# advimman/lama

Hardware: NVIDIA H100
Metric: images/sec FFCResNetGenerator @512x512 bs32 (higher is better)
Workload: dtype bf16x3(f32 accumulate)

## Files before the change

lama_b200/csrc/fft_plane_cg.cu:

```cuda
#include <stdint.h>

#include "common.cuh"
#include "fft_plane_cg.cuh"

namespace ffcb {
namespace {

using namespace fftc;

struct CgArgs {
  const float* in;  long long in_sg, in_sb;  unsigned in_sy, in_sx;
  void* spec;       long long sp_sg, sp_sb;  unsigned sp_sy, sp_sx; long long sp_lo;
  void* out;        long long out_sg, out_sb; unsigned out_sy, out_sx; long long out_lo;
  float scale;
  int hints;
  int sp_tiled;
  int out_tiled;
};

__device__ __forceinline__ uint32_t smem_addr(const void* p) { return (uint32_t)__cvta_generic_to_shared(p); }

__device__ __forceinline__ void cp_async16(uint32_t dst, const void* src, uint64_t pol) {
  asm volatile("cp.async.cg.shared.global.L2::cache_hint [%0], [%1], 16, %2;" ::"r"(dst), "l"(src), "l"(pol) : "memory");
}
__device__ __forceinline__ void cp_async_wait_all() { asm volatile("cp.async.wait_all;" ::: "memory"); }

template <int N, bool DENSE>
__global__ void __launch_bounds__(kCgThreads, CgCfg<N>::ctas_per_sm) rfft2_plane_cg_kernel(CgArgs a) {
  using Cfg = CgCfg<N>;
  constexpr unsigned WF = N / 2 + 1;
  const unsigned in_sy = DENSE ? 4u * N : a.in_sy, in_sx = DENSE ? 4u : a.in_sx;
  const unsigned sp_sy = DENSE ? 8u * WF : a.sp_sy, sp_sx = DENSE ? 8u : a.sp_sx;
  extern __shared__ __align__(16) float smem_all[];
  const int set = threadIdx.x / Cfg::set_threads, tid = threadIdx.x % Cfg::set_threads;
  const int group = blockIdx.x * Cfg::sets + set;
  float* smem = smem_all + set * Cfg::set_floats;
  float2* S = reinterpret_cast<float2*>(smem);
  {
    const float* src = a.in + (long long)group * a.in_sg + (long long)blockIdx.y * a.in_sb;
    const uint32_t base = smem_addr(smem);
    const uint64_t pol_in = l2_policy(a.hints ? 1 : 0);
#pragma unroll 8
    for (int i = 0; i < Cfg::px_iters; ++i) {
      int y, x;
      cg_pixel_slot<N>(tid, i, y, x);
      cp_async16(base + 4u * (unsigned)cg_real_idx<N>(y, x, 0), src + ((unsigned)y * in_sy + (unsigned)x * in_sx),
                 pol_in);
    }
    cp_async_wait_all();
  }
  float2* NQ = reinterpret_cast<float2*>(smem_all + Cfg::sets * Cfg::set_floats) + set * (N * 4);
  float2 v[N];
#pragma unroll 1
  for (int pass = 0; pass < 2; ++pass) {
    __syncthreads();
    if (pass == 0) {
      cg_fwd_rows_load<N>(tid, v, [&](int i) { return *reinterpret_cast<const float2*>(smem + i); });
      __syncwarp();
    } else {
      cg_fwd_cols_load<N>(tid, v, [&](int i2) { return S[i2]; });
    }
    RegFft<N>::template run<false>(v);
    if (pass == 0) {
      cg_fwd_rows_post<N>(tid, v, [&](int i2, float4 q) { *reinterpret_cast<float4*>(S + i2) = q; });
    } else {
      auto put = [&](int ky, int kx, int c, float2 z) {
        if (kx == N / 2) NQ[ky * 4 + c] = z;
        else S[cg_cplx_idx<N>(ky, kx, c)] = z;
      };
      if (tid < 32) cg_fwd_cols_post<N, true>(tid, v, put);
      else cg_fwd_cols_post<N, false>(tid, v, put);
    }
  }
  __syncthreads();
  {
    unsigned short* hi = reinterpret_cast<unsigned short*>(a.spec) + (long long)group * a.sp_sg +
                         (long long)blockIdx.y * a.sp_sb;
    const float scale = a.scale;
    const uint64_t pol_sp = l2_policy(a.hints ? 2 : 0);
    int ky, kx;
    cg_spec_pos0<N>(tid, ky, kx);
    unsigned short* tbase = reinterpret_cast<unsigned short*>(a.spec) + (long long)group * 1024;
    long long m = (long long)blockIdx.y * Cfg::positions + tid;
#pragma unroll 1
    for (int i = 0; i < Cfg::pos_iters; ++i) {
      if (ky < N) {
        const float4* src = kx == N / 2 ? reinterpret_cast<const float4*>(NQ + ky * 4)
                                        : reinterpret_cast<const float4*>(S + cg_cplx_idx<N>(ky, kx, 0));
        const float4 q0 = src[0], q1 = src[1];
        uint4 h, l;
        const float2 z0 = cscale(make_float2(q0.x, q0.y), scale), z1 = cscale(make_float2(q0.z, q0.w), scale);
        const float2 z2 = cscale(make_float2(q1.x, q1.y), scale), z3 = cscale(make_float2(q1.z, q1.w), scale);
        split_pair(z0.x, z0.y, h.x, l.x);
        split_pair(z1.x, z1.y, h.y, l.y);
        split_pair(z2.x, z2.y, h.z, l.z);
        split_pair(z3.x, z3.y, h.w, l.w);
        unsigned short* dst = a.sp_tiled ? tbase + ((m >> 7) * a.sp_sg + (m & 127) * 8)
                                         : hi + ((unsigned)ky * sp_sy + (unsigned)kx * sp_sx);
        st_hint_u4(dst, h, pol_sp);
        st_hint_u4(dst + a.sp_lo, l, pol_sp);
      }
      cg_spec_pos_next<N>(ky, kx);
      m += Cfg::set_threads;
    }
  }
}

template <int N, bool HAS_RES, bool OUT_SPLIT, bool DENSE>
__global__ void __launch_bounds__(kCgThreads, CgCfg<N>::ctas_per_sm) irfft2_plane_cg_kernel(CgArgs a) {
  using Cfg = CgCfg<N>;
  constexpr unsigned WF = N / 2 + 1;
  const unsigned in_sy = DENSE ? 4u * N : a.in_sy, in_sx = DENSE ? 4u : a.in_sx;
  const unsigned sp_sy = DENSE ? 8u * WF : a.sp_sy, sp_sx = DENSE ? 8u : a.sp_sx;
  const unsigned out_sy = DENSE ? (OUT_SPLIT ? 8u : 4u) * N : a.out_sy, out_sx = DENSE ? (OUT_SPLIT ? 8u : 4u) : a.out_sx;
  extern __shared__ __align__(16) float smem_all[];
  const int set = threadIdx.x / Cfg::set_threads, tid = threadIdx.x % Cfg::set_threads;
  const int group = blockIdx.x * Cfg::sets + set;
  float* smem = smem_all + set * Cfg::set_floats;
  float2* S = reinterpret_cast<float2*>(smem);
  {
    const float* sp = reinterpret_cast<const float*>(a.spec) + (long long)group * a.sp_sg +
                      (long long)blockIdx.y * a.sp_sb + 2 * (tid & 3);
    const uint64_t pol_sp = l2_policy(a.hints ? 1 : 0);
    auto ldz = [&](int ky, int kx) { return ld_hint_f2(sp + ((unsigned)ky * sp_sy + (unsigned)kx * sp_sx), pol_sp); };
    float2 v[N];
#pragma unroll 1
    for (int pass = 0; pass < 2; ++pass) {
      if (pass == 0) {
        if (tid < 32) cg_inv_cols_load<N, true>(tid, v, ldz);
        else cg_inv_cols_load<N, false>(tid, v, ldz);
      } else {
        __syncthreads();
        cg_inv_rows_load<N>(tid, v, [&](int i2) { return *reinterpret_cast<const float4*>(S + i2); });
        __syncwarp();
      }
      RegFft<N>::template run<true>(v);
      if (pass == 0) cg_inv_cols_post<N>(tid, v, [&](int i2, float2 z) { S[i2] = z; });
      else cg_inv_rows_post<N>(tid, v, [&](int i, float2 z) { *reinterpret_cast<float2*>(smem + i) = z; });
    }
  }
  __syncthreads();
  {
    const float* res = HAS_RES ? a.in + (long long)group * a.in_sg + (long long)blockIdx.y * a.in_sb : nullptr;
    const float scale = a.scale;
    const uint64_t pol_res = l2_policy(a.hints ? 1 : 0), pol_out = l2_policy(a.hints ? 2 : 0);
#pragma unroll 1
    for (int i0 = 0; i0 < Cfg::px_iters; i0 += 8) {
      float4 q[8];
#pragma unroll
      for (int j = 0; j < 8; ++j) {
        int y, x;
        cg_pixel_slot<N>(tid, i0 + j, y, x);
        q[j] = HAS_RES ? ld_hint_f4(res + ((unsigned)y * in_sy + (unsigned)x * in_sx), pol_res)
                       : make_float4(0.f, 0.f, 0.f, 0.f);
      }
#pragma unroll
      for (int j = 0; j < 8; ++j) {
        int y, x;
        cg_pixel_slot<N>(tid, i0 + j, y, x);
        const float4 v = *reinterpret_cast<const float4*>(smem + cg_real_idx<N>(y, x, 0));
        const float r0 = fmaf(v.x, scale, q[j].x), r1 = fmaf(v.y, scale, q[j].y);
        const float r2 = fmaf(v.z, scale, q[j].z), r3 = fmaf(v.w, scale, q[j].w);
        if constexpr (OUT_SPLIT) {
          unsigned short* hi;
          if (a.out_tiled) {
            const long long m = ((long long)blockIdx.y * N + y) * N + x;
            hi = reinterpret_cast<unsigned short*>(a.out) + ((m >> 7) * a.out_sg + (long long)(group >> 1) * 1024 +
                                                               (m & 127) * 8 + 4 * (group & 1));
          } else {
            hi = reinterpret_cast<unsigned short*>(a.out) + (long long)(group >> 1) * a.out_sg +
                 (long long)blockIdx.y * a.out_sb + 4 * (group & 1) + ((unsigned)y * out_sy + (unsigned)x * out_sx);
          }
          unsigned h0, l0, h1, l1;
          split_pair(r0, r1, h0, l0);
          split_pair(r2, r3, h1, l1);
          st_hint_v2(hi, make_uint2(h0, h1), pol_out);
          st_hint_v2(hi + a.out_lo, make_uint2(l0, l1), pol_out);
        } else {
          float* op = reinterpret_cast<float*>(a.out) + (long long)group * a.out_sg +
                      (long long)blockIdx.y * a.out_sb + ((unsigned)y * out_sy + (unsigned)x * out_sx);
          st_hint_f4(op, make_float4(r0, r1, r2, r3), pol_out);
        }
      }
    }
  }
}

bool offsets_fit(const ffcb_tensor* t) { return t->sy > 0 && t->sx > 0 && 64 * t->sy + 64 * t->sx < (1LL << 31); }

bool plane_ok(int h, int w, int c) { return (h == 64 && w == 64) || (h == 32 && w == 32 && c % 8 == 0); }

bool real_cg4(const ffcb_tensor* t) {
  return t->cg == 4 && t->fmt == FFCB_F32 && plane_ok(t->H, t->W, t->C) && t->sx % 4 == 0 && t->sy % 4 == 0 &&
         t->sb % 4 == 0 && t->sg % 4 == 0 && ((uintptr_t)t->ptr % 16) == 0 && offsets_fit(t) && t->B <= 65535;
}

}

bool plane64_cg_fwd_eligible(const ffcb_tensor* in, const ffcb_tensor* spec) {
  if (!(real_cg4(in) && spec->cg == 8 && spec->fmt == FFCB_BF16X2 && spec->lo_off % 8 == 0 &&
        ((uintptr_t)spec->ptr % 16) == 0))
    return false;
  if (spec->tile) return spec->tile == 128 && spec->sg % 8 == 0;
  return spec->sx % 8 == 0 && spec->sy % 8 == 0 && spec->sb % 8 == 0 && spec->sg % 8 == 0 && offsets_fit(spec);
}

bool plane64_cg_inv_eligible(const ffcb_tensor* spec, const ffcb_tensor* residual, const ffcb_tensor* out) {
  if (!(spec->cg == 8 && spec->fmt == FFCB_F32 && spec->sx % 2 == 0 && spec->sy % 2 == 0 && spec->sb % 2 == 0 &&
        spec->sg % 2 == 0 && ((uintptr_t)spec->ptr % 8) == 0 && offsets_fit(spec) && plane_ok(out->H, out->W, out->C) &&
        out->B <= 65535))
    return false;
  if (residual && residual->ptr && !real_cg4(residual)) return false;
  if (out->fmt == FFCB_BF16X2) {
    if (!(out->cg == 8 && out->lo_off % 4 == 0 && ((uintptr_t)out->ptr % 8) == 0 && out->C % 8 == 0)) return false;
    if (out->tile) return out->tile == 128 && out->sg % 4 == 0;
    return out->sx % 4 == 0 && out->sy % 4 == 0 && out->sb % 4 == 0 && out->sg % 4 == 0 && offsets_fit(out);
  }
  return real_cg4(out);
}

template <int N, bool DENSE>
static int launch_fwd_cg(const CgArgs& a, int groups, int batch, cudaStream_t stream) {
  using Cfg = CgCfg<N>;
  FFCB_CUDA(cudaFuncSetAttribute(rfft2_plane_cg_kernel<N, DENSE>, cudaFuncAttributeMaxDynamicSharedMemorySize,
                                 Cfg::fwd_smem_bytes));
  dim3 grid(groups / Cfg::sets, batch);
  rfft2_plane_cg_kernel<N, DENSE><<<grid, kCgThreads, Cfg::fwd_smem_bytes, stream>>>(a);
  FFCB_LAUNCH_CHECK("rfft2_plane_cg_kernel");
  return FFCB_OK;
}

static bool dense_real(const ffcb_tensor* t, int cg) { return t->sx == cg && t->sy == (int64_t)t->W * cg; }

int rfft2_plane64_cg(const ffcb_tensor* in, const ffcb_tensor* spec, cudaStream_t stream) {
  CgArgs a{};
  a.in = reinterpret_cast<const float*>(in->ptr);
  a.in_sg = in->sg; a.in_sb = in->sb; a.in_sy = (unsigned)in->sy; a.in_sx = (unsigned)in->sx;
  a.spec = spec->ptr; a.sp_sg = spec->sg; a.sp_sb = spec->sb; a.sp_sy = (unsigned)spec->sy; a.sp_sx = (unsigned)spec->sx;
  a.sp_lo = spec->lo_off;
  a.sp_tiled = spec->tile != 0;
  a.scale = 1.0f / (float)in->H;
  a.hints = l2_hints_enabled() ? 1 : 0;
  const bool dense = dense_real(in, 4) && (spec->tile != 0 || dense_real(spec, 8));
  if (in->H == 64)
    return dense ? launch_fwd_cg<64, true>(a, in->C / 4, in->B, stream) : launch_fwd_cg<64, false>(a, in->C / 4, in->B, stream);
  return dense ? launch_fwd_cg<32, true>(a, in->C / 4, in->B, stream) : launch_fwd_cg<32, false>(a, in->C / 4, in->B, stream);
}

template <int N, bool HAS_RES, bool OUT_SPLIT, bool DENSE>
static int launch_inv_cg(const CgArgs& a, int groups, int batch, cudaStream_t stream) {
  using Cfg = CgCfg<N>;
  FFCB_CUDA(cudaFuncSetAttribute(irfft2_plane_cg_kernel<N, HAS_RES, OUT_SPLIT, DENSE>,
                                 cudaFuncAttributeMaxDynamicSharedMemorySize, Cfg::smem_bytes));
  dim3 grid(groups / Cfg::sets, batch);
  irfft2_plane_cg_kernel<N, HAS_RES, OUT_SPLIT, DENSE><<<grid, kCgThreads, Cfg::smem_bytes, stream>>>(a);
  FFCB_LAUNCH_CHECK("irfft2_plane_cg_kernel");
  return FFCB_OK;
}

template <int N, bool DENSE>
static int dispatch_inv_cg(const CgArgs& a, int groups, int batch, bool has_res, bool split, cudaStream_t stream) {
  if (has_res)
    return split ? launch_inv_cg<N, true, true, DENSE>(a, groups, batch, stream)
                 : launch_inv_cg<N, true, false, DENSE>(a, groups, batch, stream);
  return split ? launch_inv_cg<N, false, true, DENSE>(a, groups, batch, stream)
               : launch_inv_cg<N, false, false, DENSE>(a, groups, batch, stream);
}

int irfft2_plane64_cg(const ffcb_tensor* spec, const ffcb_tensor* residual, const ffcb_tensor* out,
                      cudaStream_t stream) {
  const bool has_res = residual && residual->ptr;
  CgArgs a{};
  if (has_res) {
    a.in = reinterpret_cast<const float*>(residual->ptr);
    a.in_sg = residual->sg; a.in_sb = residual->sb; a.in_sy = (unsigned)residual->sy; a.in_sx = (unsigned)residual->sx;
  }
  a.spec = spec->ptr; a.sp_sg = spec->sg; a.sp_sb = spec->sb; a.sp_sy = (unsigned)spec->sy; a.sp_sx = (unsigned)spec->sx;
  a.out = out->ptr; a.out_sg = out->sg; a.out_sb = out->sb; a.out_sy = (unsigned)out->sy; a.out_sx = (unsigned)out->sx;
  a.out_lo = out->lo_off;
  a.out_tiled = out->tile != 0;
  a.scale = 1.0f / (float)out->H;
  a.hints = l2_hints_enabled() ? 1 : 0;
  const bool split = out->fmt == FFCB_BF16X2;
  const bool dense = dense_real(spec, 8) && (out->tile != 0 || dense_real(out, split ? 8 : 4)) &&
                     (!has_res || dense_real(residual, 4));
  if (out->H == 64)
    return dense ? dispatch_inv_cg<64, true>(a, out->C / 4, out->B, has_res, split, stream)
                 : dispatch_inv_cg<64, false>(a, out->C / 4, out->B, has_res, split, stream);
  return dense ? dispatch_inv_cg<32, true>(a, out->C / 4, out->B, has_res, split, stream)
               : dispatch_inv_cg<32, false>(a, out->C / 4, out->B, has_res, split, stream);
}

}
```

lama_b200/csrc/fft_plane_cg.cuh:

```cuda
#pragma once
#include "fft_core.cuh"

namespace ffcb {
namespace fftc {

constexpr int kCgThreads = 128;
template <int N> struct CgCfg {
  static constexpr int set_threads = 2 * N;
  static constexpr int sets = kCgThreads / set_threads;
  static constexpr int set_floats = N * N * 4;
  static constexpr int smem_bytes = sets * set_floats * 4;
  static constexpr int px_iters = N * N / set_threads;
  static constexpr int positions = N * (N / 2 + 1);
  static constexpr int pos_iters = (positions + set_threads - 1) / set_threads;
  static constexpr int fwd_smem_bytes = smem_bytes + sets * N * 4 * 8;
  static constexpr int ctas_per_sm = N == 64 ? 3 : 4;
};
constexpr int kCgSmemBytes = CgCfg<64>::smem_bytes;

template <int N> FFCB_HD int cg_real_idx(int y, int x, int c) { return y * (4 * N) + ((x ^ (y & 7)) << 2) + c; }
template <int N> FFCB_HD int cg_cplx_idx(int y, int k, int c) { return y * (2 * N) + ((k ^ (y & 3)) << 2) + c; }


template <int N, class Load>
FFCB_HD void cg_fwd_rows_load(int tid, float2* v, Load&& ld2) {
  const int cp = tid & 1, y = tid >> 1;
#pragma unroll
  for (int x = 0; x < N; ++x) v[x] = ld2(cg_real_idx<N>(y, x, 2 * cp));
}

template <int N, class Store>
FFCB_HD void cg_fwd_rows_post(int tid, const float2* v, Store&& st4) {
  using F = RegFft<N>;
  const int cp = tid & 1, y = tid >> 1;
#pragma unroll
  for (int k = 0; k < N / 2; ++k) {
    const float2 zk = v[F::at(k)], zm = v[F::at((N - k) & (N - 1))];
    const float2 cm = make_float2(zm.x, -zm.y), df = csub(zk, cm);
    float2 a = cscale(cadd(zk, cm), 0.5f);
    float2 b = cscale(make_float2(df.y, -df.x), 0.5f);
    if (k == 0) {
      const float2 zn = v[F::at(N / 2)];
      a = make_float2(zk.x, zn.x);
      b = make_float2(zk.y, zn.y);
    }
    st4(cg_cplx_idx<N>(y, k, 2 * cp), make_float4(a.x, a.y, b.x, b.y));
  }
}

template <int N, class Load, class Sync, class Store>
FFCB_HD void cg_fwd_rows(int tid, Load&& ld2, Sync&& sync, Store&& st4) {
  float2 v[N];
  cg_fwd_rows_load<N>(tid, v, ld2);
  sync();
  RegFft<N>::template run<false>(v);
  cg_fwd_rows_post<N>(tid, v, st4);
}

template <int N, class Load>
FFCB_HD void cg_fwd_cols_load(int tid, float2* v, Load&& ld) {
  const int c = tid & 3, kx = tid >> 2;
#pragma unroll
  for (int y = 0; y < N; ++y) v[y] = ld(cg_cplx_idx<N>(y, kx, c));
}

template <int N, bool MAYBE_PACKED, class Emit>
FFCB_HD void cg_fwd_cols_post(int tid, const float2* v, Emit&& emit) {
  using F = RegFft<N>;
  const int c = tid & 3, kx = tid >> 2;
  const bool packed = MAYBE_PACKED && kx == 0;
#pragma unroll
  for (int k = 0; k < N; ++k) {
    const float2 wk = v[F::at(k)];
    if constexpr (MAYBE_PACKED) {
      const float2 wm = v[F::at((N - k) & (N - 1))];
      const float2 cm = make_float2(wm.x, -wm.y), df = csub(wk, cm);
      const float2 x0 = cscale(cadd(wk, cm), 0.5f);
      const float2 x32 = cscale(make_float2(df.y, -df.x), 0.5f);
      emit(k, kx, c, packed ? x0 : wk);
      if (packed) emit(k, N / 2, c, x32);
    } else {
      emit(k, kx, c, wk);
    }
  }
}

template <int N, bool MAYBE_PACKED, class Load, class Emit>
FFCB_HD void cg_fwd_cols(int tid, Load&& ld, Emit&& emit) {
  float2 v[N];
  cg_fwd_cols_load<N>(tid, v, ld);
  RegFft<N>::template run<false>(v);
  cg_fwd_cols_post<N, MAYBE_PACKED>(tid, v, emit);
}

template <int N, bool MAYBE_PACKED, class Load>
FFCB_HD void cg_inv_cols_load(int tid, float2* v, Load&& ld) {
  const int kx = tid >> 2;
  const bool packed = MAYBE_PACKED && kx == 0;
#pragma unroll
  for (int k = 0; k < N; ++k) v[k] = ld(k, kx);
  if constexpr (MAYBE_PACKED) {
#pragma unroll
    for (int k = 0; k <= N / 2; ++k) {
      const int m = (N - k) & (N - 1);
      const float2 a = v[k], b = v[m];
      float2 cc = make_float2(0.f, 0.f), d = make_float2(0.f, 0.f);
      if (packed) {
        cc = ld(k, N / 2);
        d = (m != k) ? ld(m, N / 2) : cc;
      }
      const float2 h0 = cscale(cadd(a, make_float2(b.x, -b.y)), 0.5f);
      const float2 h32 = cscale(cadd(cc, make_float2(d.x, -d.y)), 0.5f);
      const float2 ih = make_float2(-h32.y, h32.x);
      const float2 lo = cadd(h0, ih), hi = csub(h0, ih);
      v[k] = packed ? lo : a;
      if (m != k) v[m] = packed ? make_float2(hi.x, -hi.y) : b;
    }
  }
}

template <int N, class Store>
FFCB_HD void cg_inv_cols_post(int tid, const float2* v, Store&& st) {
  using F = RegFft<N>;
  const int c = tid & 3, kx = tid >> 2;
#pragma unroll
  for (int y = 0; y < N; ++y) st(cg_cplx_idx<N>(y, kx, c), v[F::at(y)]);
}

template <int N, bool MAYBE_PACKED, class Load, class Store>
FFCB_HD void cg_inv_cols(int tid, Load&& ld, Store&& st) {
  float2 v[N];
  cg_inv_cols_load<N, MAYBE_PACKED>(tid, v, ld);
  RegFft<N>::template run<true>(v);
  cg_inv_cols_post<N>(tid, v, st);
}

template <int N, class Load>
FFCB_HD void cg_inv_rows_load(int tid, float2* v, Load&& ld4) {
  const int cp = tid & 1, y = tid >> 1;
#pragma unroll
  for (int k = 0; k < N / 2; ++k) {
    const float4 q = ld4(cg_cplx_idx<N>(y, k, 2 * cp));
    if (k == 0) {
      v[0] = make_float2(q.x, q.z);
      v[N / 2] = make_float2(q.y, q.w);
    } else {
      const float2 x1 = make_float2(q.x, q.y), ix2 = make_float2(-q.w, q.z), dd = csub(x1, ix2);
      v[k] = cadd(x1, ix2);
      v[N - k] = make_float2(dd.x, -dd.y);
    }
  }
}

template <int N, class Store>
FFCB_HD void cg_inv_rows_post(int tid, const float2* v, Store&& st2) {
  using F = RegFft<N>;
  const int cp = tid & 1, y = tid >> 1;
#pragma unroll
  for (int x = 0; x < N; ++x) st2(cg_real_idx<N>(y, x, 2 * cp), v[F::at(x)]);
}

template <int N, class Load, class Sync, class Store>
FFCB_HD void cg_inv_rows(int tid, Load&& ld4, Sync&& sync, Store&& st2) {
  float2 v[N];
  cg_inv_rows_load<N>(tid, v, ld4);
  sync();
  RegFft<N>::template run<true>(v);
  cg_inv_rows_post<N>(tid, v, st2);
}

template <int N>
FFCB_HD void cg_spec_pos0(int tid, int& ky, int& kx) {
  ky = tid / (N / 2 + 1);
  kx = tid % (N / 2 + 1);
}
template <int N>
FFCB_HD void cg_spec_pos_next(int& ky, int& kx) {
  constexpr int WF = N / 2 + 1, T = 2 * N;
  kx += T % WF;
  ky += T / WF;
  if (kx >= WF) { kx -= WF; ++ky; }
}

template <int N>
FFCB_HD void cg_pixel_slot(int tid, int i, int& y, int& x) {
  const int p = i * CgCfg<N>::set_threads + tid;
  y = p / N;
  x = p % N;
}

}
}
```

Baseline: 329.5.

## Make inverse plane FFT kernel persistent with L2 bulk prefetch of next spectrum

Turns the inverse FFT plane kernel into a persistent grid-stride loop over (group-set, batch) units, capped at SMs × CTAs-per-SM. Each iteration issues cp.async.bulk L2 prefetches for the current residual and the next unit's spectrum, aiming to hide global-memory latency. An extra __syncthreads is added before the shared-memory column store so buffers can be reused across iterations. The trade-off is more barriers and a fixed grid that can load-balance poorly, and the prefetch adds memory traffic on a path that may already be bandwidth-bound.

```diff
diff --git a/lama_b200/csrc/fft_plane_cg.cu b/lama_b200/csrc/fft_plane_cg.cu
--- a/lama_b200/csrc/fft_plane_cg.cu
+++ b/lama_b200/csrc/fft_plane_cg.cu
@@ -16,6 +16,9 @@
   int hints;
   int sp_tiled;
   int out_tiled;
+  int pf_spec;
+  int gx_count;
+  int units;
 };
 
 __device__ __forceinline__ uint32_t smem_addr(const void* p) { return (uint32_t)__cvta_generic_to_shared(p); }
@@ -24,6 +27,9 @@
   asm volatile("cp.async.cg.shared.global.L2::cache_hint [%0], [%1], 16, %2;" ::"r"(dst), "l"(src), "l"(pol) : "memory");
 }
 __device__ __forceinline__ void cp_async_wait_all() { asm volatile("cp.async.wait_all;" ::: "memory"); }
+__device__ __forceinline__ void prefetch_l2(const void* p, int bytes) {
+  asm volatile("cp.async.bulk.prefetch.L2.global [%0], %1;" ::"l"(p), "r"(bytes) : "memory");
+}
 
 template <int N, bool DENSE>
 __global__ void __launch_bounds__(kCgThreads, CgCfg<N>::ctas_per_sm) rfft2_plane_cg_kernel(CgArgs a) {
@@ -115,71 +121,98 @@
   const unsigned out_sy = DENSE ? (OUT_SPLIT ? 8u : 4u) * N : a.out_sy, out_sx = DENSE ? (OUT_SPLIT ? 8u : 4u) : a.out_sx;
   extern __shared__ __align__(16) float smem_all[];
   const int set = threadIdx.x / Cfg::set_threads, tid = threadIdx.x % Cfg::set_threads;
-  const int group = blockIdx.x * Cfg::sets + set;
   float* smem = smem_all + set * Cfg::set_floats;
   float2* S = reinterpret_cast<float2*>(smem);
-  {
-    const float* sp = reinterpret_cast<const float*>(a.spec) + (long long)group * a.sp_sg +
-                      (long long)blockIdx.y * a.sp_sb + 2 * (tid & 3);
-    const uint64_t pol_sp = l2_policy(a.hints ? 1 : 0);
-    auto ldz = [&](int ky, int kx) { return ld_hint_f2(sp + ((unsigned)ky * sp_sy + (unsigned)kx * sp_sx), pol_sp); };
-    float2 v[N];
-#pragma unroll 1
-    for (int pass = 0; pass < 2; ++pass) {
-      if (pass == 0) {
-        if (tid < 32) cg_inv_cols_load<N, true>(tid, v, ldz);
-        else cg_inv_cols_load<N, false>(tid, v, ldz);
-      } else {
-        __syncthreads();
-        cg_inv_rows_load<N>(tid, v, [&](int i2) { return *reinterpret_cast<const float4*>(S + i2); });
-        __syncwarp();
-      }
-      RegFft<N>::template run<true>(v);
-      if (pass == 0) cg_inv_cols_post<N>(tid, v, [&](int i2, float2 z) { S[i2] = z; });
-      else cg_inv_rows_post<N>(tid, v, [&](int i, float2 z) { *reinterpret_cast<float2*>(smem + i) = z; });
-    }
-  }
-  __syncthreads();
-  {
-    const float* res = HAS_RES ? a.in + (long long)group * a.in_sg + (long long)blockIdx.y * a.in_sb : nullptr;
-    const float scale = a.scale;
-    const uint64_t pol_res = l2_policy(a.hints ? 1 : 0), pol_out = l2_policy(a.hints ? 2 : 0);
-#pragma unroll 1
-    for (int i0 = 0; i0 < Cfg::px_iters; i0 += 8) {
-      float4 q[8];
+  auto spec_of = [&](int u) {
+    int gx, b;
+    cg_unit(u, a.gx_count, gx, b);
+    return reinterpret_cast<const float*>(a.spec) + (long long)(gx * Cfg::sets + set) * a.sp_sg + (long long)b * a.sp_sb;
+  };
+#pragma unroll 1
+  for (int u = blockIdx.x; u < a.units; u += gridDim.x) {
+    const int next = u + gridDim.x;
+    int gx, b;
+    cg_unit(u, a.gx_count, gx, b);
+    const int group = gx * Cfg::sets + set;
+    const float* res = HAS_RES ? a.in + (long long)group * a.in_sg + (long long)b * a.in_sb : nullptr;
+    if (DENSE && tid < kCgPrefetchChunks) {
+      int off, bytes;
+      if (HAS_RES) {
+        cg_prefetch_chunk(tid, Cfg::real_set_bytes, off, bytes);
+        prefetch_l2(reinterpret_cast<const char*>(res) + off, bytes);
+      }
+      if (a.pf_spec && next < a.units) {
+        cg_prefetch_chunk(tid, Cfg::spec_set_bytes, off, bytes);
+        prefetch_l2(reinterpret_cast<const char*>(spec_of(next)) + off, bytes);
+      }
+    }
+    {
+      const float* sp0 = spec_of(u) + 2 * (tid & 3);
+      const uint64_t pol_sp = l2_policy(a.hints ? 1 : 0);
+      float2 v[N];
+#pragma unroll 1
+      for (int pass = 0; pass < 2; ++pass) {
+        if (pass == 0) {
+          const float* sp = sp0;
+          asm volatile("" : "+l"(sp));
+          auto ldz = [&](int ky, int kx) { return ld_hint_f2(sp + ((unsigned)ky * sp_sy + (unsigned)kx * sp_sx), pol_sp); };
+          if (tid < 32) cg_inv_cols_load<N, true>(tid, v, ldz);
+          else cg_inv_cols_load<N, false>(tid, v, ldz);
+        } else {
+          __syncthreads();
+          cg_inv_rows_load<N>(tid, v, [&](int i2) { return *reinterpret_cast<const float4*>(S + i2); });
+          __syncwarp();
+        }
+        RegFft<N>::template run<true>(v);
+        if (pass == 0) {
+          __syncthreads();
+          cg_inv_cols_post<N>(tid, v, [&](int i2, float2 z) { S[i2] = z; });
+        } else {
+          cg_inv_rows_post<N>(tid, v, [&](int i, float2 z) { *reinterpret_cast<float2*>(smem + i) = z; });
+        }
+      }
+    }
+    __syncthreads();
+    {
+      const float scale = a.scale;
+      const uint64_t pol_res = l2_policy(a.hints ? 1 : 0), pol_out = l2_policy(a.hints ? 2 : 0);
+#pragma unroll 1
+      for (int i0 = 0; i0 < Cfg::px_iters; i0 += 8) {
+        float4 q[8];
 #pragma unroll
-      for (int j = 0; j < 8; ++j) {
-        int y, x;
-        cg_pixel_slot<N>(tid, i0 + j, y, x);
-        q[j] = HAS_RES ? ld_hint_f4(res + ((unsigned)y * in_sy + (unsigned)x * in_sx), pol_res)
-                       : make_float4(0.f, 0.f, 0.f, 0.f);
-      }
+        for (int j = 0; j < 8; ++j) {
+          int y, x;
+          cg_pixel_slot<N>(tid, i0 + j, y, x);
+          q[j] = HAS_RES ? ld_hint_f4(res + ((unsigned)y * in_sy + (unsigned)x * in_sx), pol_res)
+                         : make_float4(0.f, 0.f, 0.f, 0.f);
+        }
 #pragma unroll
-      for (int j = 0; j < 8; ++j) {
-        int y, x;
-        cg_pixel_slot<N>(tid, i0 + j, y, x);
-        const float4 v = *reinterpret_cast<const float4*>(smem + cg_real_idx<N>(y, x, 0));
-        const float r0 = fmaf(v.x, scale, q[j].x), r1 = fmaf(v.y, scale, q[j].y);
-        const float r2 = fmaf(v.z, scale, q[j].z), r3 = fmaf(v.w, scale, q[j].w);
-        if constexpr (OUT_SPLIT) {
-          unsigned short* hi;
-          if (a.out_tiled) {
-            const long long m = ((long long)blockIdx.y * N + y) * N + x;
-            hi = reinterpret_cast<unsigned short*>(a.out) + ((m >> 7) * a.out_sg + (long long)(group >> 1) * 1024 +
-                                                               (m & 127) * 8 + 4 * (group & 1));
+        for (int j = 0; j < 8; ++j) {
+          int y, x;
+          cg_pixel_slot<N>(tid, i0 + j, y, x);
+          const float4 v = *reinterpret_cast<const float4*>(smem + cg_real_idx<N>(y, x, 0));
+          const float r0 = fmaf(v.x, scale, q[j].x), r1 = fmaf(v.y, scale, q[j].y);
+          const float r2 = fmaf(v.z, scale, q[j].z), r3 = fmaf(v.w, scale, q[j].w);
+          if constexpr (OUT_SPLIT) {
+            unsigned short* hi;
+            if (a.out_tiled) {
+              const long long m = ((long long)b * N + y) * N + x;
+              hi = reinterpret_cast<unsigned short*>(a.out) + ((m >> 7) * a.out_sg + (long long)(group >> 1) * 1024 +
+                                                                 (m & 127) * 8 + 4 * (group & 1));
+            } else {
+              hi = reinterpret_cast<unsigned short*>(a.out) + (long long)(group >> 1) * a.out_sg +
+                   (long long)b * a.out_sb + 4 * (group & 1) + ((unsigned)y * out_sy + (unsigned)x * out_sx);
+            }
+            unsigned h0, l0, h1, l1;
+            split_pair(r0, r1, h0, l0);
+            split_pair(r2, r3, h1, l1);
+            st_hint_v2(hi, make_uint2(h0, h1), pol_out);
+            st_hint_v2(hi + a.out_lo, make_uint2(l0, l1), pol_out);
           } else {
-            hi = reinterpret_cast<unsigned short*>(a.out) + (long long)(group >> 1) * a.out_sg +
-                 (long long)blockIdx.y * a.out_sb + 4 * (group & 1) + ((unsigned)y * out_sy + (unsigned)x * out_sx);
+            float* op = reinterpret_cast<float*>(a.out) + (long long)group * a.out_sg +
+                        (long long)b * a.out_sb + ((unsigned)y * out_sy + (unsigned)x * out_sx);
+            st_hint_f4(op, make_float4(r0, r1, r2, r3), pol_out);
           }
-          unsigned h0, l0, h1, l1;
-          split_pair(r0, r1, h0, l0);
-          split_pair(r2, r3, h1, l1);
-          st_hint_v2(hi, make_uint2(h0, h1), pol_out);
-          st_hint_v2(hi + a.out_lo, make_uint2(l0, l1), pol_out);
-        } else {
-          float* op = reinterpret_cast<float*>(a.out) + (long long)group * a.out_sg +
-                      (long long)blockIdx.y * a.out_sb + ((unsigned)y * out_sy + (unsigned)x * out_sx);
-          st_hint_f4(op, make_float4(r0, r1, r2, r3), pol_out);
         }
       }
     }
@@ -217,6 +250,15 @@
     return out->sx % 4 == 0 && out->sy % 4 == 0 && out->sb % 4 == 0 && out->sg % 4 == 0 && offsets_fit(out);
   }
   return real_cg4(out);
+}
+
+static int persistent_grid(CgArgs& a, int groups, int batch, int sets, int ctas_per_sm) {
+  int dev = 0, sms = 132;
+  FFCB_CUDA(cudaGetDevice(&dev));
+  FFCB_CUDA(cudaDeviceGetAttribute(&sms, cudaDevAttrMultiProcessorCount, dev));
+  a.gx_count = groups / sets;
+  a.units = a.gx_count * batch;
+  return cg_grid(a.units, sms, ctas_per_sm);
 }
 
 template <int N, bool DENSE>
@@ -248,11 +290,11 @@
 }
 
 template <int N, bool HAS_RES, bool OUT_SPLIT, bool DENSE>
-static int launch_inv_cg(const CgArgs& a, int groups, int batch, cudaStream_t stream) {
+static int launch_inv_cg(CgArgs a, int groups, int batch, cudaStream_t stream) {
   using Cfg = CgCfg<N>;
   FFCB_CUDA(cudaFuncSetAttribute(irfft2_plane_cg_kernel<N, HAS_RES, OUT_SPLIT, DENSE>,
                                  cudaFuncAttributeMaxDynamicSharedMemorySize, Cfg::smem_bytes));
-  dim3 grid(groups / Cfg::sets, batch);
+  const int grid = persistent_grid(a, groups, batch, Cfg::sets, Cfg::ctas_per_sm);
   irfft2_plane_cg_kernel<N, HAS_RES, OUT_SPLIT, DENSE><<<grid, kCgThreads, Cfg::smem_bytes, stream>>>(a);
   FFCB_LAUNCH_CHECK("irfft2_plane_cg_kernel");
   return FFCB_OK;
@@ -279,6 +321,7 @@
   a.out = out->ptr; a.out_sg = out->sg; a.out_sb = out->sb; a.out_sy = (unsigned)out->sy; a.out_sx = (unsigned)out->sx;
   a.out_lo = out->lo_off;
   a.out_tiled = out->tile != 0;
+  a.pf_spec = ((uintptr_t)spec->ptr % 16) == 0 && spec->sg % 4 == 0 && spec->sb % 4 == 0;
   a.scale = 1.0f / (float)out->H;
   a.hints = l2_hints_enabled() ? 1 : 0;
   const bool split = out->fmt == FFCB_BF16X2;
diff --git a/lama_b200/csrc/fft_plane_cg.cuh b/lama_b200/csrc/fft_plane_cg.cuh
--- a/lama_b200/csrc/fft_plane_cg.cuh
+++ b/lama_b200/csrc/fft_plane_cg.cuh
@@ -15,6 +15,8 @@
   static constexpr int pos_iters = (positions + set_threads - 1) / set_threads;
   static constexpr int fwd_smem_bytes = smem_bytes + sets * N * 4 * 8;
   static constexpr int ctas_per_sm = N == 64 ? 3 : 4;
+  static constexpr int real_set_bytes = N * N * 16;
+  static constexpr int spec_set_bytes = positions * 32;
 };
 constexpr int kCgSmemBytes = CgCfg<64>::smem_bytes;
 
@@ -182,6 +184,23 @@
   if (kx >= WF) { kx -= WF; ++ky; }
 }
 
+FFCB_HD int cg_grid(int units, int sms, int ctas_per_sm) {
+  return units < sms * ctas_per_sm ? units : sms * ctas_per_sm;
+}
+FFCB_HD void cg_unit(int u, int gx_count, int& gx, int& b) {
+  gx = u % gx_count;
+  b = u / gx_count;
+}
+constexpr int kCgPrefetchChunks = 4;
+FFCB_HD void cg_prefetch_chunk(int i, int set_bytes, int& off, int& bytes) {
+  bytes = set_bytes / kCgPrefetchChunks;
+  off = i * bytes;
+}
+static_assert(CgCfg<64>::real_set_bytes % (16 * kCgPrefetchChunks) == 0 &&
+              CgCfg<64>::spec_set_bytes % (16 * kCgPrefetchChunks) == 0 &&
+              CgCfg<32>::real_set_bytes % (16 * kCgPrefetchChunks) == 0 &&
+              CgCfg<32>::spec_set_bytes % (16 * kCgPrefetchChunks) == 0, "prefetch chunks must be 16-byte multiples");
+
 template <int N>
 FFCB_HD void cg_pixel_slot(int tid, int i, int& y, int& x) {
   const int p = i * CgCfg<N>::set_threads + tid;
```

Result: no change. 332.3, median of 6 (+0.9%).
